# prsinha1/Distributed-Inverse-Problem-Admm

Hardware: AMD Instinct MI355X
Metric: ADMM node-updates/sec (whole node), 512² phantom; rel-Fro vs CPU ref (higher is better)
Workload: dtype f32 samples / f64 state; 1 GPU; C3 (BASELINE.json configs[2] 512^2, 16 graph nodes (ring), 96 angles/node, float32 samples, iso TV, lam=0.02 rho=2, split-Bregman 10x5 CG) on 1 GPU(s), one step = one outer ADMM iteration; image=512, nodes=16, angles_per_node=96, graph=ring, parallelism=graph-node shards x1, batch_streams=1

## Files before the change

### distributed-inverse-problem-admm_amd/csrc/admm_tomo.hip

```cpp
#include <hip/hip_runtime.h>

#include <algorithm>
#include <cmath>
#include <cstdio>
#include <cstdlib>
#include <cstring>
#include <string>
#include <type_traits>
#include <utility>
#include <vector>

#include "../../include/admm_tomo.h"
#include "kernels.hpp"

using namespace admm;

namespace {
thread_local std::string g_err;

int fail(int code, const std::string& msg) {
  g_err = msg;
  return code;
}

// ... 64 lines not shown
  double Kb = 0.0;
  int kbias = 0;
  int wexp = 0;
  FgGroup* groups = nullptr;
  FgRange* rng = nullptr;
  int n_groups = 0;
  static constexpr int kPlans = 6;
  FgGroup* plan_groups[kPlans] = {};
  FgRange* plan_rng[kPlans] = {};
  int plan_n[kPlans] = {}, plan_blocks[kPlans] = {};
  double plan_staged[kPlans] = {};
  std::vector<int4> plan_blk[kPlans];
  std::vector<char> plan_caseA[kPlans];
  bool mirror_half = false;
  Buf fg_order;
  int fg_nblk = 0, fg_order_nch = 0;
  int fg_cpb = 1;
  hipStream_t cap = nullptr;

  bool csr = false;
  long long nnz = 0;
  Buf f_ptr, f_idx, f_val, t_ptr, t_idx, t_val;

  Buf op_img, op_imgT, op_sino, op_fpart;
  Buf op_order[kPlans];
  int op_nblk[kPlans] = {};
  int op_fpart_key = -1;

  bool bound = false;
  admm_batch b{};
  int vb = 1;
  bool mm = false;
  int bk_staging = 0;
  int n_cu = 0;
  admm_ctx* half = nullptr;
  Buf xs, xsT, p, pT, Hp, sino, bI, fpart, r, c, d2, e2;
  Buf dsumS;
  Buf x2, p2;
  Buf pring;
  Buf ats;
  std::vector<hipEvent_t>* tf_ev = nullptr;
  size_t tf_next = 0;
  int tf_kind = 0;
  bool ats_valid = false;
  hipGraph_t g_update_reuse = nullptr;
  hipGraphExec_t x_update_reuse = nullptr;
  Buf partH, partS, partD, partE;
  Buf redH;
  int P_back = 0, P_tile = 0, P_fwd = 0, P_edge = 0;
  hipGraph_t g_update = nullptr, g_cons = nullptr;
  hipGraphExec_t x_update = nullptr, x_cons = nullptr;
};

namespace {

#define RET(expr)                   \
  do {                              \
    int _rc = (expr);               \
    if (_rc != ADMM_OK) return _rc; \
  } while (0)

constexpr int kXcds = 8;

int vb_for(int V, int dtype) {
  const int vb = V >= 5 ? 8 : (V >= 3 ? 4 : (V == 2 ? 2 : 1));
  return dtype == ADMM_DTYPE_F64 ? std::min(vb, 4) : vb;
// ... 260 lines not shown
  }
  dim3 cg((C->mrays + kBlock - 1) / kBlock, nch);
  hipLaunchKernelGGL((k_fwd_combine<T, VB, MODE>), cg, dim3(kBlock), 0, s, (const T*)C->fpart.p, sino, b, part,
                     C->fang, C->g.n_det, C->g.n_angles, V);
  CHECK_LAUNCH();
  return ADMM_OK;
}

template <typename T, int VB, int MODE>
int launch_back(admm_ctx* C, BackArgs<T> a, int V, hipStream_t s) {
  if constexpr (MODE == BACK_H || MODE == BACK_INIT || MODE == BACK_DIAG || MODE == BACK_ATB) {
    if (C->mm) {
      constexpr int VBV = mirror_vb<T, VB>(), MH = VBV / 2;
      const admm_ctx* H = C->half;
      a.ang = H->bang;
      a.angc = H->bangc;
      a.K = H->Kb;
      a.kbias = H->kbias;
      a.wexp = H->wexp;
      a.N = C->g.N;
      a.n_det = C->g.n_det;
      a.n_ang = H->g.n_angles;
      a.V = V;
      const int N = C->g.N, Nh = (N + 1) / 2;
      dim3 grid((N + kBTJ - 1) / kBTJ, (Nh + kBTI - 1) / kBTI, ((V + VB - 1) / VB) * (VB / MH));
      bool done = false;
      if constexpr (back_mirror_dma<T, VBV, MODE>()) {
        if (C->bk_staging == 1) {
          hipLaunchKernelGGL((k_back_mirror_reg<T, VBV, VB, MODE>), grid, dim3(kBkThreads), 0, s, a);
          done = true;
        } else if constexpr (std::is_same<T, float>::value && ADMM_BK_LB2) {
          const bool fills = (long)grid.x * grid.y * grid.z >= 2L * C->n_cu;
          if (grid.z % 2 == 0 && (C->bk_staging == 3 || (C->bk_staging == 0 && fills))) {
            hipLaunchKernelGGL((k_back_mirror_2<T, VBV, VB>), dim3(grid.x, grid.y, grid.z / 2), dim3(kBkThreads), 0,
                               s, a);
            done = true;
          }
        }
      }
      if (!done) hipLaunchKernelGGL((k_back_mirror<T, VBV, VB, MODE>), grid, dim3(kBkThreads), 0, s, a);
      CHECK_LAUNCH();
      return ADMM_OK;
    }
  }
  a.ang = C->bang;
  a.angc = C->bangc;
  a.K = C->Kb;
  a.kbias = C->kbias;
  a.wexp = C->wexp;
  a.N = C->g.N;
  a.n_det = C->g.n_det;
  a.n_ang = C->g.n_angles;
  a.V = V;
  const int N = C->g.N;
  dim3 grid((N + kBTJ - 1) / kBTJ, (N + kBTI - 1) / kBTI, MODE == BACK_WSQ ? 1 : (V + VB - 1) / VB);
  if (C->csr) {
    a.csr_ptr = (const int*)C->t_ptr.p;
    a.csr_idx = (const int*)C->t_idx.p;
    a.csr_val = (const T*)C->t_val.p;
    hipLaunchKernelGGL((k_back<T, VB, MODE, true>), grid, dim3(kBkThreads), 0, s, a);
  } else {
    hipLaunchKernelGGL((k_back<T, VB, MODE>), grid, dim3(kBkThreads), 0, s, a);
  }
  CHECK_LAUNCH();
  return ADMM_OK;
}

int back_partitions(admm_ctx* C) {
// ... 344 lines not shown
}

extern "C" {

int admm_abi_version(void) { return ADMM_ABI_VERSION; }
const char* admm_last_error(void) { return g_err.c_str(); }

int admm_ctx_create(admm_ctx** out, const admm_geom* geom, int dtype, int max_images, int device) {
  if (!out || !geom) return fail(ADMM_E_INVALID, "null argument");
  *out = nullptr;
  const admm_geom g = *geom;
  if (g.N < 2 || g.n_angles < 1 || g.n_det < 1) return fail(ADMM_E_INVALID, "bad geometry sizes");
  if (g.N > 4096) return fail(ADMM_E_INVALID, "N > 4096 is not supported");
  if (dtype != ADMM_DTYPE_F32 && dtype != ADMM_DTYPE_F64) return fail(ADMM_E_INVALID, "bad dtype");
  if (max_images < 1) return fail(ADMM_E_INVALID, "max_images < 1");
  const double h = 2.0 / g.N;
  const double hd = (g.det_max - g.det_min) / g.n_det;
  if (!(hd > 0)) return fail(ADMM_E_INVALID, "det_max <= det_min");
  if (hd < h * (1.0 - 1e-9))
    return fail(ADMM_E_INVALID, "detector spacing finer than the pixel size is not supported "
                                "(det_width_factor must be >= 1 with n_det = N)");
  const size_t npix = (size_t)g.N * g.N, m = (size_t)g.n_angles * g.n_det;
  if ((size_t)max_images * npix * 8 >= (1ull << 31) || (size_t)max_images * m * 8 >= (1ull << 31))
    return fail(ADMM_E_INVALID, "batch too large for 32-bit buffer offsets; split it across contexts");
  DEVICE_SCOPE(device);
  admm_ctx* C = new admm_ctx();
  C->g = g;
  C->dtype = dtype;
  C->device = device;
  {
    const char* st = getenv("ADMM_BK_STAGING");
    const std::string v = st ? st : "";
    C->bk_staging = v == "reg" ? 1 : v == "dma1" ? 2 : v == "dma2" ? 3 : 0;
  }
  HIPCHK(hipDeviceGetAttribute(&C->n_cu, hipDeviceAttributeMultiprocessorCount, device));
  C->max_images = max_images;
  C->npix = (int)npix;
  C->mrays = (int)m;

  std::vector<FwdAngle> fa(g.n_angles);
  std::vector<BackAngle> ba(g.n_angles);
  std::vector<BackAngleC> bc(g.n_angles);
  C->Kb = -g.det_min / hd - 0.5;
  const double c0 = 0.5 * (g.N - 1);
  for (int t = 0; t < g.n_angles; ++t) {
    const double th = g.angle_min + (t + 0.5) * (g.angle_max - g.angle_min) / g.n_angles;
    const double cs = std::cos(th), sn = std::sin(th);
    const bool caseA = std::fabs(cs) >= std::fabs(sn);
    const double al = caseA ? cs : sn, be = caseA ? sn : cs;
    fa[t].A0 = c0 + (g.det_min / h + 0.5 * hd / h + c0 * be) / al;
    fa[t].A1 = (hd / h) / al;
    fa[t].dl = -be / al;
    fa[t].L = h / std::fabs(al);
    fa[t].caseA = caseA ? 1 : 0;
    ba[t].Bi = cs * h / hd;
    ba[t].Bj = sn * h / hd;
    ba[t].B0 = -c0 * (ba[t].Bi + ba[t].Bj) - g.det_min / hd - 0.5;
    ba[t].slope = (hd / h) / std::fabs(al);
    ba[t].L = h / std::fabs(al);
    bc[t].Bi = ba[t].Bi;
    bc[t].Bj = ba[t].Bj;
    const float sLf = (float)(ba[t].slope * ba[t].L);
    bc[t].ws = float2v{-sLf, sLf};
    bc[t].wc = float2v{(float)ba[t].L, (float)(ba[t].L - ba[t].slope * ba[t].L)};
    while (std::ldexp((double)bc[t].wc.x, -C->wexp) > 1.0) ++C->wexp;
    const double kmn = C->Kb - c0 * (std::fabs(ba[t].Bi) + std::fabs(ba[t].Bj));
// ... 406 lines not shown
  RET(ensure(C->dsumS, Vp * npix * ds));
  RET(ensure(C->x2, (size_t)V * npix * 8));
  RET(ensure(C->p2, Vp * npix * ds));
  if (B.cg_iters > 1 && B.cg_iters <= kMaxCgRing)
    RET(ensure(C->pring, (size_t)(B.cg_iters - 1) * Vp * npix * ds));
  if (B.flags & ADMM_BATCH_KEEP_X) RET(ensure(C->ats, Vp * npix * ds));
  C->ats_valid = false;
  RET(ensure(C->sino, Vp * m * ds));
  RET(ensure(C->bI, Vp * m * ds));
  RET(ensure(C->r, V * npix * 8));
  RET(ensure(C->c, V * npix * 8));
  RET(ensure(C->d2, 2 * V * npix * 8));
  RET(ensure(C->e2, 2 * V * npix * 8));
  C->P_back = back_partitions(C);
  const int N = C->g.N;
  C->P_tile = ((N + kTile - 1) / kTile) * ((N + kTile - 1) / kTile);
  if ((size_t)Vp * npix * ds >= (1ull << 31) || (size_t)Vp * m * ds >= (1ull << 31))
    return fail(ADMM_E_INVALID, "batch too large for 32-bit buffer offsets");
  C->P_fwd = C->mm ? (int)((C->half->mrays + kBlock - 1) / kBlock)
           : (C->n_groups > 0 || C->csr) ? (int)((m + kBlock - 1) / kBlock)
                                         : ((C->g.n_det + kFwdRays - 1) / kFwdRays) * C->g.n_angles;
  C->P_edge = B.z ? (int)((npix + kBlock * 4 - 1) / (kBlock * 4)) : (int)((npix + kConsPix - 1) / kConsPix);
  RET(ensure(C->partH, (size_t)5 * V * C->P_back * 8));
  RET(ensure(C->partS, (size_t)V * C->P_fwd * 8));
  RET(ensure(C->partD, (size_t)5 * V * C->P_back * 8));
  RET(ensure(C->partE, (size_t)3 * std::max(1, B.n_edges) * C->P_edge * 8));
  RET(ensure(C->redH, (size_t)5 * V * 8 * std::max(1, std::min(B.cg_iters, kMaxCgRing))));
  C->bound = true;
  RET(with_vb(C->vb, [&](auto vbc) {
    constexpr int VB = decltype(vbc)::value;
    const int nch = (V + VB - 1) / VB;
    if (C->dtype == ADMM_DTYPE_F32)
      hipLaunchKernelGGL((k_pack_d<float, VB>), dim3((unsigned)((npix + 255) / 256), nch), dim3(256), 0, C->cap,
                         B.dsum, (float*)C->dsumS.p, (int)npix, V);
    else
      hipLaunchKernelGGL((k_pack_d<double, VB>), dim3((unsigned)((npix + 255) / 256), nch), dim3(256), 0, C->cap,
                         B.dsum, (double*)C->dsumS.p, (int)npix, V);
    CHECK_LAUNCH();
    return ADMM_OK;
  }));
  HIPCHK(hipStreamSynchronize(C->cap));
  auto fu = [&](hipStream_t s) {
    return C->dtype == ADMM_DTYPE_F32 ? enqueue_update_any<float>(C, s) : enqueue_update_any<double>(C, s);
  };
  RET(capture(C, fu, &C->g_update, &C->x_update));
  if (B.flags & ADMM_BATCH_KEEP_X) {
    auto fr = [&](hipStream_t s) {
      return C->dtype == ADMM_DTYPE_F32 ? enqueue_update_any<float>(C, s, true)
                                        : enqueue_update_any<double>(C, s, true);
    };
    RET(capture(C, fr, &C->g_update_reuse, &C->x_update_reuse));
  }
  if (B.n_edges > 0) {
    auto fc = [&](hipStream_t s) { return enqueue_consensus(C, s); };
    RET(capture(C, fc, &C->g_cons, &C->x_cons));
  }
  HIPCHK(hipDeviceSynchronize());
  return ADMM_OK;
}

extern "C++" {
template <typename T>
int batch_atb(admm_ctx* C, double* atb_out, hipStream_t s) {
  const int V = C->b.V;
  return with_vb(C->vb, [&](auto vbc) {
    constexpr int VB = decltype(vbc)::value;
    const int nch = (V + VB - 1) / VB;
    hipLaunchKernelGGL((k_pack<T, VB>), dim3((C->mrays + 255) / 256, nch), dim3(256), 0, s, (const T*)C->b.b,
                       (T*)C->bI.p, C->mrays, V);
    CHECK_LAUNCH();
// ... 172 lines not shown
```

### distributed-inverse-problem-admm_amd/csrc/kernels.hpp

```cpp
#pragma once
#include <hip/hip_runtime.h>
#include <stdint.h>

#include <type_traits>

namespace admm {

constexpr int kBlock = 256;
constexpr int kTile = 32;
constexpr int kFwdRays = 64;
constexpr int kFwdSegs = 8;
constexpr int kFwdBlock = kFwdRays * kFwdSegs;

struct FwdAngle {
  double A0, A1, dl;
  double L;
  int caseA;
  int pad;
};
struct BackAngle {
  double B0, Bi, Bj;
  double slope, L;
};

// ... 1064 lines not shown
  const double c = x[i * N + j];
  gx = (i < N - 1) ? x[(i + 1) * N + j] - c : 0.0;
  gy = (j < N - 1) ? x[i * N + j + 1] - c : 0.0;
}

__device__ __forceinline__ void tv_sub(double gx, double gy, int kind, double& px, double& py) {
  if (kind == 0) {
    const double m = sqrt(gx * gx + gy * gy);
    if (m > 1e-12) {
      px = gx / m;
      py = gy / m;
    } else {
      px = 0.0;
      py = 0.0;
    }
  } else {
    px = fabs(gx) > 1e-12 ? copysign(1.0, gx) : 0.0;
    py = fabs(gy) > 1e-12 ? copysign(1.0, gy) : 0.0;
  }
}

__device__ __forceinline__ double kt_w_at(const double* __restrict__ d, const double* __restrict__ e, int N,
                                          int i, int j) {
  const int n = N * N;
  double s = 0.0;
  const int o = i * N + j;
  if (i >= 1) s += d[o - N] - e[o - N];
  if (i <= N - 2) s -= d[o] - e[o];
  if (j >= 1) s += d[n + o - 1] - e[n + o - 1];
  if (j <= N - 2) s -= d[n + o] - e[n + o];
  return s;
}

template <typename T, int VB, int MODE, int NQ, int VS = VB, bool ACC = false>
__device__ __forceinline__ void back_epilogue(const BackArgs<T>& A, int i, int j, int chunk, int v0, int nv,
                                              const T (&acc)[VB], double (&pq)[VB][NQ], int lo = 0) {
  const int N = A.N;
  const int npix = N * N;
  const int pix = i * N + j;
  const size_t sbase = (size_t)chunk * npix * VS + lo;
  if constexpr (MODE == BACK_PLAIN) {
    gstore<T, VB>(A.out_t + sbase + (size_t)pix * VS, acc);
  } else if constexpr (MODE == BACK_ATB) {
#pragma unroll
    for (int u = 0; u < VB; ++u)
      if (u < nv) A.out_d[(size_t)(v0 + u) * npix + pix] = (double)acc[u];
  } else if constexpr (MODE == BACK_WSQ) {
    A.out_d[pix] = fmax((double)acc[0], 1e-12);
  } else if constexpr (MODE == BACK_H && std::is_same<T, float>::value) {
    using F2 = float2v;
    constexpr int NP = VB / 2;
    const T* pv = A.pin + sbase;
    T pc[VB], pn[VB], dv[VB], outv[VB];
    F2 kt2[NP > 0 ? NP : 1], pc2[NP > 0 ? NP : 1];
    float kt1 = 0.0f;
    gload<T, VB>(pv + (size_t)pix * VS, pc);
#pragma unroll
    for (int h = 0; h < NP; ++h) {
      pc2[h] = F2{pc[2 * h], pc[2 * h + 1]};
      kt2[h] = F2{0.0f, 0.0f};
    }
    auto nb = [&](size_t o, bool sub_pc_first) {
      gload<T, VB>(pv + o * VS, pn);
#pragma unroll
      for (int h = 0; h < NP; ++h) {
        const F2 q = F2{pn[2 * h], pn[2 * h + 1]};
        kt2[h] = sub_pc_first ? kt2[h] + (pc2[h] - q) : kt2[h] - (q - pc2[h]);
      }
      if constexpr (VB % 2) kt1 = sub_pc_first ? kt1 + (pc[VB - 1] - pn[VB - 1]) : kt1 - (pn[VB - 1] - pc[VB - 1]);
    };
    if (i >= 1) nb((size_t)(pix - N), true);
    if (i <= N - 2) nb((size_t)(pix + N), false);
    if (j >= 1) nb((size_t)(pix - 1), true);
    if (j <= N - 2) nb((size_t)(pix + 1), false);
    gload<T, VB>(A.dsum_s + sbase + (size_t)pix * VS, dv);
    const float rf = (float)A.rho, mf = (float)A.mu;
    const F2 rho2 = F2{rf, rf}, mu2 = F2{mf, mf};
#pragma unroll
    for (int h = 0; h < NP; ++h) {
      const F2 d2 = F2{dv[2 * h], dv[2 * h + 1]} * rho2;
      F2 hv = __builtin_elementwise_fma(d2, pc2[h], F2{acc[2 * h], acc[2 * h + 1]});
      hv = __builtin_elementwise_fma(mu2, kt2[h], hv);
      outv[2 * h] = hv.x;
      outv[2 * h + 1] = hv.y;
    }
    if constexpr (VB % 2) outv[VB - 1] = fmaf(mf, kt1, fmaf(dv[VB - 1] * rf, pc[VB - 1], acc[VB - 1]));
#pragma unroll
    for (int u = 0; u < VB; ++u) {
      if (u >= nv) outv[u] = T(0);
      if (u < nv) {
        const double hd = (double)outv[u], pcd = (double)pc[u];
        const double rv = A.r[(size_t)(v0 + u) * npix + pix];
        pq[u][0] = fma(pcd, hd, ACC ? pq[u][0] : 0.0);
        pq[u][1] = fma(rv, hd, ACC ? pq[u][1] : 0.0);
        pq[u][2] = fma(hd, hd, ACC ? pq[u][2] : 0.0);
        pq[u][3] = fma(rv, rv, ACC ? pq[u][3] : 0.0);
        pq[u][4] = fma(rv, pcd, ACC ? pq[u][4] : 0.0);
      }
    }
    gstore<T, VB>(A.out_t + sbase + (size_t)pix * VS, outv);
  } else if constexpr (MODE == BACK_H || MODE == BACK_INIT) {
    const T* pv = A.pin + sbase;
    T pc[VB], pn[VB];
    double ktk[VB];
    gload<T, VB>(pv + (size_t)pix * VS, pc);
    if (i >= 1) {
      gload<T, VB>(pv + (size_t)(pix - N) * VS, pn);
#pragma unroll
      for (int u = 0; u < VB; ++u) ktk[u] = (double)pc[u] - (double)pn[u];
    } else {
#pragma unroll
      for (int u = 0; u < VB; ++u) ktk[u] = 0.0;
    }
    if (i <= N - 2) {
      gload<T, VB>(pv + (size_t)(pix + N) * VS, pn);
#pragma unroll
      for (int u = 0; u < VB; ++u) ktk[u] -= (double)pn[u] - (double)pc[u];
    }
    if (j >= 1) {
      gload<T, VB>(pv + (size_t)(pix - 1) * VS, pn);
#pragma unroll
      for (int u = 0; u < VB; ++u) ktk[u] += (double)pc[u] - (double)pn[u];
    }
    if (j <= N - 2) {
      gload<T, VB>(pv + (size_t)(pix + 1) * VS, pn);
#pragma unroll
      for (int u = 0; u < VB; ++u) ktk[u] -= (double)pn[u] - (double)pc[u];
    }
    T outv[VB], dv[VB];
    if constexpr (MODE == BACK_H) gload<T, VB>(A.dsum_s + sbase + (size_t)pix * VS, dv);
#pragma unroll
    for (int u = 0; u < VB; ++u) {
      outv[u] = T(0);
      if (u < nv) {
        const size_t vo = (size_t)(v0 + u) * npix;
        const double pcd = (double)pc[u];
        const double dd = (MODE == BACK_H) ? (double)dv[u] : A.dsum[vo + pix];
        const double h = (double)acc[u] + A.rho * dd * pcd + A.mu * ktk[u];
        if constexpr (MODE == BACK_H) {
          const T hp = (T)h;
          outv[u] = hp;
          const double hd = (double)hp;
          const double rv = A.r[vo + pix];
          if constexpr (ACC) {
            pq[u][0] += pcd * hd;
            pq[u][1] += rv * hd;
            pq[u][2] += hd * hd;
            pq[u][3] += rv * rv;
            pq[u][4] += rv * pcd;
          } else {
            pq[u][0] = pcd * hd;
            pq[u][1] = rv * hd;
            pq[u][2] = hd * hd;
            pq[u][3] = rv * rv;
            pq[u][4] = rv * pcd;
          }
        } else {
          const double* dv = A.dvar + 2 * vo;
          const double* ev = A.evar + 2 * vo;
          const double rr = A.atb[vo + pix] + A.rho * A.cvec[vo + pix] + A.mu * kt_w_at(dv, ev, N, i, j) - h;
          A.out_d[vo + pix] = rr;
          outv[u] = (T)rr;
        }
      }
    }
    gstore<T, VB>(A.out_t + sbase + (size_t)pix * VS, outv);
  }
}

#ifndef ADMM_BK_TI
#define ADMM_BK_TI 32
// ... 347 lines not shown
  for (int u = 0; u < VB; ++u)
#pragma unroll
    for (int q = 0; q < NQ; ++q) pq[u][q] = 0.0;
  if constexpr (MODE == BACK_DIAG) {
    __shared__ double diag_s[kDiagScratch];
    diag_epilogue_tile<T, VB>(A, diag_s, ib, jb, i, j, inb, chunk, v0, nv, acc, pq);
  } else if (inb) {
    back_epilogue<T, VB, MODE, NQ>(A, i, j, chunk, v0, nv, acc, pq);
  }

  if constexpr (MODE == BACK_H || MODE == BACK_DIAG) {
    constexpr int NT = VB * NQ, NS = RsShape<NT>::NS;
    __shared__ double lds[kBkWaves * NS];
    __shared__ double tot[NS];
    double flat[NT];
#pragma unroll
    for (int u = 0; u < VB; ++u)
#pragma unroll
      for (int q = 0; q < NQ; ++q) flat[u * NQ + q] = pq[u][q];
    block_reduce_flat<NT, kBkWaves>(flat, lds, tot);
    const int t = threadIdx.x;
    if (t < VB * NQ && t / NQ < nv) {
      const int P = gridDim.x * gridDim.y;
      const int b = blockIdx.y * gridDim.x + blockIdx.x;
      A.part[((size_t)v0 * NQ + t) * P + b] = tot[t];
    }
  }
}

template <typename T, int VB, int MODE>
constexpr bool back_mirror_dma() {
  return ADMM_BK_DMA && MODE == BACK_H && Planes<T, VB>::NPL == 2 && sizeof(Pack<T, Planes<T, VB>::PV>) == 16;
}
template <typename T, int VB, int VBR, int MODE, bool DMAQ>
__device__ __forceinline__ void back_mirror_body(const BackArgs<T>& A) {
  static_assert(MODE == BACK_H || MODE == BACK_INIT || MODE == BACK_DIAG || MODE == BACK_ATB, "batch modes");
  constexpr int MH = VB / 2, MS = VBR / MH;
  static_assert(VB % 2 == 0 && VBR % MH == 0, "mirror: VB = 2 x (a divisor of VBR)");
  constexpr int NQ = (MODE == BACK_H || MODE == BACK_DIAG) ? 5 : 1;
  constexpr int NPL = Planes<T, VB>::NPL, PV = Planes<T, VB>::PV;
  constexpr int PB = (int)sizeof(Pack<T, PV>);
  const int N = A.N, n_det = A.n_det, n_ang = A.n_ang;
  const int Nh = (N + 1) / 2;
  const size_t m_full = (size_t)2 * n_ang * n_det;
  const int jb = blockIdx.x * kBTJ, ib = blockIdx.y * kBTI;
  const int lane = threadIdx.x & 63, wv = threadIdx.x >> 6;
  const int j = jb + 16 * (wv % kBkPatchJ) + (lane & 15);
  const int i = ib + 4 * (wv / kBkPatchJ) + (lane >> 4);
  const int i2 = N - 1 - i;
  const bool inb = (i < Nh) && (j < N);
  const bool inb2 = inb && (i2 != i);
  const int chunk = blockIdx.z, rc = chunk / MS, mq = chunk % MS;
  const int v0 = rc * VBR + mq * MH;
  const int nv = min(MH, A.V - v0);
  const double c0 = 0.5 * (N - 1);
  const double xi = (double)min(i, Nh - 1) - c0, yj = (double)min(j, N - 1) - c0;
  const int jhi = min(jb + kBTJ - 1, N - 1), ihi = min(ib + kBTI - 1, Nh - 1);
  const int kbias = A.kbias;
  const double Kc = A.K + (double)kbias;
  const double Kcb = Kc + kKfBias;
  constexpr bool FB = std::is_same<T, float>::value;
  constexpr int ANGC_ = ((NPL > 2) ? kBAngC / 2 : kBAngC) / 2;
  constexpr int ANGC_DIAG = (98304 / (2 * NPL * kBWin * PB)) & ~3;
  constexpr int ANGC = (MODE == BACK_DIAG && ANGC_ > ANGC_DIAG) ? ANGC_DIAG : ANGC_;
  static_assert(ANGC % 4 == 0 && ANGC >= 4, "angle chunks are read as int4 groups");
  constexpr bool DMA = DMAQ && back_mirror_dma<T, VB, MODE>();
  constexpr int NWB = DMA ? 4 : 2, NKS = DMA ? 3 : 2;
  constexpr int BUFB = 2 * NPL * ANGC * kBWin * PB;
  __shared__ Pack<T, PV> win[NWB][NPL][ANGC][kBWin];
  __shared__ int4 kmin_s[NKS][2][ANGC / 4 + 1];
  __shared__ int kst_s[DMA ? 3 : 1][2][DMA ? ANGC + 1 : 1];
  T acc1[VB], acc2[VB];
#pragma unroll
  for (int u = 0; u < VB; ++u) acc1[u] = acc2[u] = T(0);
  const T* sino_c = A.sino + (size_t)rc * m_full * VBR + mq * MH;
  int t0c = 0;

  auto kmin_load = [&](int t0) {
    const BackAngleC& g = A.angc[min(t0 + ((int)threadIdx.x % ANGC), n_ang - 1)];
    return make_double2(g.Bi, g.Bj);
  };
  auto kmin_store = [&](int buf, double2 bij, int bo = 0) {
    const int w = (int)threadIdx.x / ANGC;
    const double xa = (double)ib - c0, xb = (double)ihi - c0;
    const double x0 = w ? -xb : xa, x1 = w ? -xa : xb;
    auto kf = [&](double xx, int jj) { return fma(xx, bij.x, fma((double)jj - c0, bij.y, Kc)); };
    const double kmn = fmin(fmin(kf(x0, jb), kf(x0, jhi)), fmin(kf(x1, jb), kf(x1, jhi)));
    const int a = (int)threadIdx.x % ANGC;
    const int k0w = (int)floor(kmn) - 1;
    int koff = (a * kBWin - k0w) * PB;
    if constexpr (FB) koff = (int)((unsigned)koff - kKfHi * (unsigned)PB);
    if constexpr (DMA) {
      koff = (int)((unsigned)koff + (unsigned)bo);
      kst_s[buf][min(w, 1)][w < 2 ? a : ANGC] = k0w - kbias;
    }
    reinterpret_cast<int*>(kmin_s[buf][min(w, 1)])[w < 2 ? a : ANGC] = koff;
  };
  auto kmin_chunk = [&](int t0, int buf) { kmin_store(buf, kmin_load(t0)); };
  auto kmin_chunk_b = [&](int t0, int buf, int bo) { kmin_store(buf, kmin_load(t0), bo); };
  constexpr int NE = 2 * ANGC * kBWin * NPL;
  constexpr int SPER = (NE + kBkThreads - 1) / kBkThreads;
// ... 178 lines not shown
      chunk_taps(t0, nt, kb);
      if (t0 + ANGC < n_ang) {
        __syncthreads();
        wcommit(t0 + ANGC);
        kmin_store(kb, rec2);
        __syncthreads();
      }
    }
  }
  if constexpr (std::is_same<T, float>::value) {
    if (A.wexp != 0) {
#pragma unroll
      for (int u = 0; u < VB; ++u) {
        acc1[u] = ldexpf(acc1[u], A.wexp);
        acc2[u] = ldexpf(acc2[u], A.wexp);
      }
    }
  }
  T r1[MH], r2[MH];
#pragma unroll
  for (int h = 0; h < MH; ++h) {
    r1[h] = acc1[h] + acc2[MH + h];
    r2[h] = acc2[h] + acc1[MH + h];
  }
  double pq[MH][NQ];
#pragma unroll
  for (int u = 0; u < MH; ++u)
#pragma unroll
    for (int q = 0; q < NQ; ++q) pq[u][q] = 0.0;
  if constexpr (MODE == BACK_DIAG) {
    __shared__ double diag_s[kDiagScratch];
    diag_epilogue_tile<T, MH, VBR>(A, diag_s, ib, jb, i, j, inb, rc, v0, nv, r1, pq, mq * MH);
    diag_epilogue_tile<T, MH, VBR>(A, diag_s, N - ib - kBTI, jb, i2, j, inb2, rc, v0, nv, r2, pq, mq * MH);
  } else {
    if (inb) back_epilogue<T, MH, MODE, NQ, VBR>(A, i, j, rc, v0, nv, r1, pq, mq * MH);
    if (inb2) back_epilogue<T, MH, MODE, NQ, VBR, true>(A, i2, j, rc, v0, nv, r2, pq, mq * MH);
  }
  if constexpr (MODE == BACK_H || MODE == BACK_DIAG) {
    constexpr int NT = MH * NQ, NS = RsShape<NT>::NS;
    __shared__ double lds[kBkWaves * NS];
    __shared__ double tot[NS];
    double flat[NT];
#pragma unroll
    for (int u = 0; u < MH; ++u)
#pragma unroll
      for (int q = 0; q < NQ; ++q) flat[u * NQ + q] = pq[u][q];
    block_reduce_flat<NT, kBkWaves>(flat, lds, tot);
    const int t = threadIdx.x;
    if (t < MH * NQ && t / NQ < nv) {
      const int P = gridDim.x * gridDim.y;
      const int b = blockIdx.y * gridDim.x + blockIdx.x;
      A.part[((size_t)v0 * NQ + t) * P + b] = tot[t];
    }
  }
}

template <typename T, int VB, int VBR, int MODE>
__global__ __launch_bounds__(kBkThreads) void k_back_mirror(BackArgs<T> A) {
  back_mirror_body<T, VB, VBR, MODE, true>(A);
}
template <typename T, int VB, int VBR, int MODE>
__global__ __launch_bounds__(kBkThreads) void k_back_mirror_reg(BackArgs<T> A) {
  back_mirror_body<T, VB, VBR, MODE, false>(A);
}

template <typename T, int VB, int VBR>
__global__ __launch_bounds__(kBkThreads) void k_back_mirror_2(BackArgs<T> A) {
  constexpr int MODE = BACK_H, NQ = 5, LB = 2;
  constexpr int MH = VB / 2, MS = VBR / MH;
  static_assert(VB % 2 == 0 && VBR % MH == 0, "mirror: VB = 2 x (a divisor of VBR)");
  constexpr int NPL = Planes<T, VB>::NPL, PV = Planes<T, VB>::PV;
  constexpr int PB = (int)sizeof(Pack<T, PV>);
  static_assert(std::is_same<T, float>::value && NPL == 2 && PB == 16, "float32 16-byte window packs");
  const int N = A.N, n_det = A.n_det, n_ang = A.n_ang;
  const int Nh = (N + 1) / 2;
  const size_t m_full = (size_t)2 * n_ang * n_det;
  const int jb = blockIdx.x * kBTJ, ib = blockIdx.y * kBTI;
  const int lane = threadIdx.x & 63, wv = threadIdx.x >> 6;
  const int j = jb + 16 * (wv % kBkPatchJ) + (lane & 15);
  const int i = ib + 4 * (wv / kBkPatchJ) + (lane >> 4);
  const int i2 = N - 1 - i;
  const bool inb = (i < Nh) && (j < N);
  const bool inb2 = inb && (i2 != i);
  const double c0 = 0.5 * (N - 1);
  const double xi = (double)min(i, Nh - 1) - c0, yj = (double)min(j, N - 1) - c0;
  const int jhi = min(jb + kBTJ - 1, N - 1), ihi = min(ib + kBTI - 1, Nh - 1);
  const int kbias = A.kbias;
  const double Kc = A.K + (double)kbias;
  const double Kcb = Kc + kKfBias;
  constexpr int ANGC = kBAngC / 4;
  static_assert(ANGC % 4 == 0 && ANGC >= 4, "angle chunks are read as int4 groups");
  constexpr int WINB = 2 * NPL * ANGC * kBWin * PB;
  constexpr int BUFB = LB * WINB;
  __shared__ Pack<T, PV> win[2 * LB * 2][NPL][ANGC][kBWin];
  __shared__ int4 kmin_s[3][2][ANGC / 4 + 1];
  __shared__ int kst_s[3][2][ANGC + 1];
  T acc1[LB][VB], acc2[LB][VB];
#pragma unroll
  for (int l = 0; l < LB; ++l)
#pragma unroll
    for (int u = 0; u < VB; ++u) acc1[l][u] = acc2[l][u] = T(0);

  auto kmin_load = [&](int t0) {
    const BackAngleC& g = A.angc[min(t0 + ((int)threadIdx.x % ANGC), n_ang - 1)];
    return make_double2(g.Bi, g.Bj);
  };
  auto kmin_store = [&](int ks, double2 bij, int bo) {
    const int w = (int)threadIdx.x / ANGC;
    const double xa = (double)ib - c0, xb = (double)ihi - c0;
    const double x0 = w ? -xb : xa, x1 = w ? -xa : xb;
    auto kf = [&](double xx, int jj) { return fma(xx, bij.x, fma((double)jj - c0, bij.y, Kc)); };
    const double kmn = fmin(fmin(kf(x0, jb), kf(x0, jhi)), fmin(kf(x1, jb), kf(x1, jhi)));
    const int a = (int)threadIdx.x % ANGC;
    const int k0w = (int)floor(kmn) - 1;
    const int koff = (int)((unsigned)((a * kBWin - k0w) * PB) - kKfHi * (unsigned)PB + (unsigned)bo);
    kst_s[ks][min(w, 1)][w < 2 ? a : ANGC] = k0w - kbias;
    reinterpret_cast<int*>(kmin_s[ks][min(w, 1)])[w < 2 ? a : ANGC] = koff;
  };
  constexpr int NE = LB * 2 * ANGC * kBWin * NPL;
  constexpr int NI = NE / (64 * kBkWaves);
  static_assert(NE % (64 * kBkWaves) == 0 && (ANGC * kBWin) % 64 == 0, "whole pieces, one (lane block, window, plane) each");
  const int wvu = __builtin_amdgcn_readfirstlane(wv);
  auto dma = [&](int t0, int ks, int bo) {
    const int nt = min(ANGC, n_ang - t0);
#pragma unroll
    for (int e = 0; e < NI; ++e) {
// ... 64 lines not shown
#pragma unroll
      for (int u = 0; u < 4; ++u) g[u] = rec(gq + u);
      const int4 k1 = kmin_s[ks][0][tt >> 2], k2 = kmin_s[ks][1][tt >> 2];
      tap2(g[0], k1.x, k2.x);
      tap2(g[1], k1.y, k2.y);
      tap2(g[2], k1.z, k2.z);
      tap2(g[3], k1.w, k2.w);
    }
    for (; tt < nt; ++tt)
      tap2(rec(gq + (tt & 3)), reinterpret_cast<const int*>(kmin_s[ks][0])[tt],
           reinterpret_cast<const int*>(kmin_s[ks][1])[tt]);
  };
  kmin_store(0, kmin_load(0), 0);
  if (ANGC < n_ang) kmin_store(1, kmin_load(ANGC), BUFB);
  __syncthreads();
  dma(0, 0, 0);
  __syncthreads();
  for (int t0 = 0, ci = 0, ks = 0; t0 < n_ang; t0 += ANGC, ++ci, ks = ks == 2 ? 0 : ks + 1) {
    const int nt = min(ANGC, n_ang - t0);
    const double2 rec2 = kmin_load(min(t0 + 2 * ANGC, n_ang - 1));
    const int ks1 = ks == 2 ? 0 : ks + 1, ks2 = ks1 == 2 ? 0 : ks1 + 1;
    if (t0 + ANGC < n_ang) dma(t0 + ANGC, ks1, (ci & 1) ? 0 : BUFB);
    chunk_taps(t0, nt, ks);
    if (t0 + ANGC < n_ang) {
      if (t0 + 2 * ANGC < n_ang) kmin_store(ks2, rec2, (ci & 1) ? BUFB : 0);
      __syncthreads();
    }
  }
  constexpr int NT = MH * NQ, NS = RsShape<NT>::NS;
  __shared__ double lds[kBkWaves * NS];
  __shared__ double tot[NS];
  const int P = gridDim.x * gridDim.y;
  const int b = blockIdx.y * gridDim.x + blockIdx.x;
#pragma unroll
  for (int l = 0; l < LB; ++l) {
    if (A.wexp != 0) {
#pragma unroll
      for (int u = 0; u < VB; ++u) {
        acc1[l][u] = ldexpf(acc1[l][u], A.wexp);
        acc2[l][u] = ldexpf(acc2[l][u], A.wexp);
      }
    }
    T r1[MH], r2[MH];
#pragma unroll
    for (int h = 0; h < MH; ++h) {
      r1[h] = acc1[l][h] + acc2[l][MH + h];
      r2[h] = acc2[l][h] + acc1[l][MH + h];
    }
    double pq[MH][NQ];
#pragma unroll
    for (int u = 0; u < MH; ++u)
#pragma unroll
      for (int q = 0; q < NQ; ++q) pq[u][q] = 0.0;
    const int z = (int)blockIdx.z * LB + l, rc = z / MS, mq = z % MS;
    const int v0 = rc * VBR + mq * MH, nv = min(MH, A.V - v0);
    if (inb) back_epilogue<T, MH, MODE, NQ, VBR>(A, i, j, rc, v0, nv, r1, pq, mq * MH);
    if (inb2) back_epilogue<T, MH, MODE, NQ, VBR, true>(A, i2, j, rc, v0, nv, r2, pq, mq * MH);
    double flat[NT];
#pragma unroll
    for (int u = 0; u < MH; ++u)
#pragma unroll
      for (int q = 0; q < NQ; ++q) flat[u * NQ + q] = pq[u][q];
    block_reduce_flat<NT, kBkWaves>(flat, lds, tot);
    const int t = threadIdx.x;
    if (t < NT && t / NQ < nv) A.part[((size_t)v0 * NQ + t) * P + b] = tot[t];
  }
}

template <int VB>
struct EwMap {
  static constexpr int TI = kTile / VB;
  static constexpr int RPI = 8 / VB;
  int u, jj, isub;
  __device__ EwMap() : u(threadIdx.x % VB), jj((threadIdx.x / VB) % kTile), isub(threadIdx.x / (kTile * VB)) {}
};

template <typename T, int VB>
struct TileT {
  T t[EwMap<VB>::TI][kTile + 1][VB];
};

template <typename T, int VB>
__device__ __forceinline__ void tile_store_T(TileT<T, VB>& tl, T* __restrict__ outT, int N, int i0, int j0) {
  constexpr int TI = EwMap<VB>::TI;
  __syncthreads();
  const int u = threadIdx.x % VB, r = (threadIdx.x / VB) % TI, c0 = threadIdx.x / (VB * TI);
  for (int c = c0; c < kTile; c += kBlock / (VB * TI)) {
    const int jj = j0 + c, ii = i0 + r;
    if (jj < N && ii < N) outT[((size_t)jj * N + ii) * VB + u] = tl.t[r][c][u];
  }
}

template <typename T, int VB>
__global__ __launch_bounds__(kBlock) void k_start_reuse(
    const T* __restrict__ ats, const double* __restrict__ x, EdgeIn E, const double* __restrict__ q,
    const int* __restrict__ inc_off, const int* __restrict__ inc_edge, const int* __restrict__ inc_qslot,
    const int* __restrict__ inc_sign, const double* __restrict__ atb, double* __restrict__ cvec,
    const double* __restrict__ dsum, const double* __restrict__ dvar, const double* __restrict__ evar,
    double* __restrict__ r, T* __restrict__ p, T* __restrict__ pT, double rho, double mu, int N, int V) {
  constexpr int ROWS = kBlock / kTile;
  __shared__ T tl[ROWS][kTile + 1][VB];
  const int chunk = blockIdx.z, v0 = chunk * VB, nv = min(VB, V - v0);
  const int npix = N * N;
  const size_t sbase = (size_t)chunk * npix * VB;
  const int jj = threadIdx.x % kTile, ii = threadIdx.x / kTile;
  const int i0 = blockIdx.y * ROWS, j0 = blockIdx.x * kTile;
  const int i = i0 + ii, j = j0 + jj;
  if (i < N && j < N) {
    const int pix = i * N + j;
    T av[VB], outv[VB];
    gload<T, VB>(ats + sbase + (size_t)pix * VB, av);
#pragma unroll
    for (int u = 0; u < VB; ++u) {
      outv[u] = T(0);
      if (u < nv) {
        const int v = v0 + u;
        const size_t vo = (size_t)v * npix;
        const double* xv = x + vo;
        double cc = 0.0;
        for (int qq = inc_off[v]; qq < inc_off[v + 1]; ++qq) {
          const double vij = edge_v(E, inc_edge[qq], inc_sign[qq], npix, pix);
          cc += q[(size_t)inc_qslot[qq] * npix + pix] * vij;
        }
        cvec[vo + pix] = cc;
        const double pcd = (double)(T)xv[pix];
        double ktk = 0.0;
        if (i >= 1) ktk += pcd - (double)(T)xv[pix - N];
        if (i <= N - 2) ktk -= (double)(T)xv[pix + N] - pcd;
        if (j >= 1) ktk += pcd - (double)(T)xv[pix - 1];
        if (j <= N - 2) ktk -= (double)(T)xv[pix + 1] - pcd;
        const double ab = atb[vo + pix];
        const double h = ((double)av[u] + ab) + rho * dsum[vo + pix] * pcd + mu * ktk;
        const double rr = ab + rho * cc + mu * kt_w_at(dvar + 2 * vo, evar + 2 * vo, N, i, j) - h;
        r[vo + pix] = rr;
        outv[u] = (T)rr;
      }
      tl[ii][jj][u] = outv[u];
    }
    gstore<T, VB>(p + sbase + (size_t)pix * VB, outv);
  }
  __syncthreads();
  const int u = threadIdx.x % VB, rr_ = (threadIdx.x / VB) % ROWS, c0 = threadIdx.x / (VB * ROWS);
  for (int c = c0; c < kTile; c += kBlock / (VB * ROWS)) {
    const int jc = j0 + c, ic = i0 + rr_;
    if (jc < N && ic < N) pT[sbase + ((size_t)jc * N + ic) * VB + u] = tl[rr_][c][u];
  }
}

template <typename T, int VB>
__global__ __launch_bounds__(kBlock) void k_gather(const double* __restrict__ x, EdgeIn E,
                                                   const double* __restrict__ q,
                                                   const int* __restrict__ inc_off, const int* __restrict__ inc_edge,
                                                   const int* __restrict__ inc_qslot,
                                                   const int* __restrict__ inc_sign, double* __restrict__ c,
                                                   T* __restrict__ xs, T* __restrict__ xsT, int N, int V) {
  __shared__ TileT<T, VB> tl;
  const EwMap<VB> mp;
  const int chunk = blockIdx.z, v = chunk * VB + mp.u;
  const bool live = v < V;
  const int npix = N * N;
  const size_t sbase = (size_t)chunk * npix * VB;
  const int i0 = blockIdx.y * EwMap<VB>::TI, j0 = blockIdx.x * kTile;
  const int e0 = live ? inc_off[v] : 0, e1 = live ? inc_off[v + 1] : 0;
// ... 316 lines not shown
    T sv = T(0);
    if (live) {
      double gx, gy, ux, uy, ndx, ndy, e0, e1;
      if constexpr (UIN) {
        const double u0 = din[2 * vo + o], u1 = din[2 * vo + npix + o];
        double d0, d1;
        shrink2(u0, u1, tau, kind, d0, d1);
        e0 = u0 - d0;
        e1 = u1 - d1;
      } else {
        e0 = ev[o];
        e1 = ev[npix + o];
      }
      gradx(mp.u, xv, i, j, gx, gy);
      ux = gx + e0;
      uy = gy + e1;
      shrink2(ux, uy, tau, kind, ndx, ndy);
      const double nex = ux - ndx, ney = uy - ndy;
      dout[2 * vo + o] = ndx;
      dout[2 * vo + npix + o] = ndy;
      eout[2 * vo + o] = nex;
      eout[2 * vo + npix + o] = ney;
      const double xn = xat(mp.u, xv, i, j);
      if constexpr (FUSE) xout[vo + o] = xn;
      sv = (T)xn;
    }
    p[sbase + (size_t)o * VB + mp.u] = sv;
    tl.t[rw][mp.jj][mp.u] = sv;
  }
  tv_tile_store_T<T, VB>(tl, pT + sbase, N, i0, j0);
}

template <typename T, int VB>
__global__ void k_pack_d(const double* __restrict__ in, T* __restrict__ out, int L, int V) {
  const int q = blockIdx.x * blockDim.x + threadIdx.x;
  const int chunk = blockIdx.y, v0 = chunk * VB;
  if (q >= L) return;
  T s[VB];
#pragma unroll
  for (int u = 0; u < VB; ++u) s[u] = (v0 + u < V) ? (T)in[(size_t)(v0 + u) * L + q] : T(0);
  gstore<T, VB>(out + ((size_t)chunk * L + q) * VB, s);
}

template <typename T, int VB>
__global__ void k_pack(const T* __restrict__ in, T* __restrict__ out, int L, int V) {
  const int q = blockIdx.x * blockDim.x + threadIdx.x;
  const int chunk = blockIdx.y, v0 = chunk * VB;
  if (q >= L) return;
  T s[VB];
#pragma unroll
  for (int u = 0; u < VB; ++u) s[u] = (v0 + u < V) ? in[(size_t)(v0 + u) * L + q] : T(0);
  gstore<T, VB>(out + ((size_t)chunk * L + q) * VB, s);
}

template <typename T, int VB>
__global__ void k_unpack(const T* __restrict__ in, T* __restrict__ out, int L, int V) {
  const int q = blockIdx.x * blockDim.x + threadIdx.x;
  const int chunk = blockIdx.y, v0 = chunk * VB;
  if (q >= L) return;
  T s[VB];
  gload<T, VB>(in + ((size_t)chunk * L + q) * VB, s);
#pragma unroll
  for (int u = 0; u < VB; ++u)
    if (v0 + u < V) out[(size_t)(v0 + u) * L + q] = s[u];
}

template <bool WEIGHTED>
__global__ __launch_bounds__(kBlock) void k_consensus(const double* __restrict__ xext, double* __restrict__ y,
                                                      double* __restrict__ yb, double* __restrict__ z,
                                                      const double* __restrict__ w,
                                                      const int* __restrict__ ea, const int* __restrict__ eb,
                                                      double* __restrict__ part, int npix, int e0 = 0) {
  __shared__ double lds[12];
// ... 177 lines not shown
```

Before: 2237 node-updates/s.

## Stage backprojection epilogue p-tiles and start-reuse x halos in LDS; prescale dsum by rho

```diff
diff --git a/distributed-inverse-problem-admm_amd/csrc/admm_tomo.hip b/distributed-inverse-problem-admm_amd/csrc/admm_tomo.hip
--- a/distributed-inverse-problem-admm_amd/csrc/admm_tomo.hip
+++ b/distributed-inverse-problem-admm_amd/csrc/admm_tomo.hip
@@ -120,6 +120,7 @@
   int vb = 1;
   bool mm = false;
   int bk_staging = 0;
+  bool bk_epi_lds = true;
   int n_cu = 0;
   admm_ctx* half = nullptr;
   Buf xs, xsT, p, pT, Hp, sino, bI, fpart, r, c, d2, e2;
@@ -446,8 +447,18 @@
         } else if constexpr (std::is_same<T, float>::value && ADMM_BK_LB2) {
           const bool fills = (long)grid.x * grid.y * grid.z >= 2L * C->n_cu;
           if (grid.z % 2 == 0 && (C->bk_staging == 3 || (C->bk_staging == 0 && fills))) {
-            hipLaunchKernelGGL((k_back_mirror_2<T, VBV, VB>), dim3(grid.x, grid.y, grid.z / 2), dim3(kBkThreads), 0,
-                               s, a);
+            if (C->bk_epi_lds)
+              hipLaunchKernelGGL((k_back_mirror_2<T, VBV, VB>), dim3(grid.x, grid.y, grid.z / 2),
+                                 dim3(kBkThreads), 0, s, a);
+            else
+              hipLaunchKernelGGL((k_back_mirror_2_gepi<T, VBV, VB>), dim3(grid.x, grid.y, grid.z / 2),
+                                 dim3(kBkThreads), 0, s, a);
+            done = true;
+          }
+        }
+        if constexpr (std::is_same<T, float>::value) {
+          if (!done && !C->bk_epi_lds) {
+            hipLaunchKernelGGL((k_back_mirror_gepi<T, VBV, VB, MODE>), grid, dim3(kBkThreads), 0, s, a);
             done = true;
           }
         }
@@ -858,6 +869,8 @@
     const char* st = getenv("ADMM_BK_STAGING");
     const std::string v = st ? st : "";
     C->bk_staging = v == "reg" ? 1 : v == "dma1" ? 2 : v == "dma2" ? 3 : 0;
+    const char* ep = getenv("ADMM_BK_EPI");
+    C->bk_epi_lds = !(ep && std::string(ep) == "global");
   }
   HIPCHK(hipDeviceGetAttribute(&C->n_cu, hipDeviceAttributeMultiprocessorCount, device));
   C->max_images = max_images;
@@ -1330,10 +1343,10 @@
     const int nch = (V + VB - 1) / VB;
     if (C->dtype == ADMM_DTYPE_F32)
       hipLaunchKernelGGL((k_pack_d<float, VB>), dim3((unsigned)((npix + 255) / 256), nch), dim3(256), 0, C->cap,
-                         B.dsum, (float*)C->dsumS.p, (int)npix, V);
+                         B.dsum, (float*)C->dsumS.p, (int)npix, V, B.rho);
     else
       hipLaunchKernelGGL((k_pack_d<double, VB>), dim3((unsigned)((npix + 255) / 256), nch), dim3(256), 0, C->cap,
-                         B.dsum, (double*)C->dsumS.p, (int)npix, V);
+                         B.dsum, (double*)C->dsumS.p, (int)npix, V, B.rho);
     CHECK_LAUNCH();
     return ADMM_OK;
   }));
diff --git a/distributed-inverse-problem-admm_amd/csrc/kernels.hpp b/distributed-inverse-problem-admm_amd/csrc/kernels.hpp
--- a/distributed-inverse-problem-admm_amd/csrc/kernels.hpp
+++ b/distributed-inverse-problem-admm_amd/csrc/kernels.hpp
@@ -1120,9 +1120,24 @@
   return s;
 }
 
-template <typename T, int VB, int MODE, int NQ, int VS = VB, bool ACC = false>
+struct PGlobal {};
+template <typename T, int VB, int PITCH>
+struct PTile {
+  static_assert(sizeof(Pack<T, VB>) == 16, "one 16-byte slot per pixel");
+  const __attribute__((address_space(3))) char* base;
+  int i0, j0;
+  __device__ __forceinline__ void load(int i, int j, T (&o)[VB]) const {
+    typedef unsigned int u32x4 __attribute__((ext_vector_type(4)));
+    const u32x4 k =
+        *reinterpret_cast<const __attribute__((address_space(3))) u32x4*>(base + ((i - i0) * PITCH + (j - j0)) * 16);
+    __builtin_memcpy(o, &k, 16);
+  }
+};
+
+template <typename T, int VB, int MODE, int NQ, int VS = VB, bool ACC = false, class PSrc = PGlobal>
 __device__ __forceinline__ void back_epilogue(const BackArgs<T>& A, int i, int j, int chunk, int v0, int nv,
-                                              const T (&acc)[VB], double (&pq)[VB][NQ], int lo = 0) {
+                                              const T (&acc)[VB], double (&pq)[VB][NQ], int lo = 0,
+                                              PSrc psrc = PSrc{}) {
   const int N = A.N;
   const int npix = N * N;
   const int pix = i * N + j;
@@ -1142,14 +1157,20 @@
     T pc[VB], pn[VB], dv[VB], outv[VB];
     F2 kt2[NP > 0 ? NP : 1], pc2[NP > 0 ? NP : 1];
     float kt1 = 0.0f;
-    gload<T, VB>(pv + (size_t)pix * VS, pc);
+    auto ldp = [&](int ii, int jj, T(&o)[VB]) {
+      if constexpr (std::is_same<PSrc, PGlobal>::value)
+        gload<T, VB>(pv + (size_t)(ii * N + jj) * VS, o);
+      else
+        psrc.load(ii, jj, o);
+    };
+    ldp(i, j, pc);
 #pragma unroll
     for (int h = 0; h < NP; ++h) {
       pc2[h] = F2{pc[2 * h], pc[2 * h + 1]};
       kt2[h] = F2{0.0f, 0.0f};
     }
-    auto nb = [&](size_t o, bool sub_pc_first) {
-      gload<T, VB>(pv + o * VS, pn);
+    auto nb = [&](int ii, int jj, bool sub_pc_first) {
+      ldp(ii, jj, pn);
 #pragma unroll
       for (int h = 0; h < NP; ++h) {
         const F2 q = F2{pn[2 * h], pn[2 * h + 1]};
@@ -1157,22 +1178,22 @@
       }
       if constexpr (VB % 2) kt1 = sub_pc_first ? kt1 + (pc[VB - 1] - pn[VB - 1]) : kt1 - (pn[VB - 1] - pc[VB - 1]);
     };
-    if (i >= 1) nb((size_t)(pix - N), true);
-    if (i <= N - 2) nb((size_t)(pix + N), false);
-    if (j >= 1) nb((size_t)(pix - 1), true);
-    if (j <= N - 2) nb((size_t)(pix + 1), false);
+    if (i >= 1) nb(i - 1, j, true);
+    if (i <= N - 2) nb(i + 1, j, false);
+    if (j >= 1) nb(i, j - 1, true);
+    if (j <= N - 2) nb(i, j + 1, false);
     gload<T, VB>(A.dsum_s + sbase + (size_t)pix * VS, dv);
-    const float rf = (float)A.rho, mf = (float)A.mu;
-    const F2 rho2 = F2{rf, rf}, mu2 = F2{mf, mf};
+    const float mf = (float)A.mu;
+    const F2 mu2 = F2{mf, mf};
 #pragma unroll
     for (int h = 0; h < NP; ++h) {
-      const F2 d2 = F2{dv[2 * h], dv[2 * h + 1]} * rho2;
+      const F2 d2 = F2{dv[2 * h], dv[2 * h + 1]};
       F2 hv = __builtin_elementwise_fma(d2, pc2[h], F2{acc[2 * h], acc[2 * h + 1]});
       hv = __builtin_elementwise_fma(mu2, kt2[h], hv);
       outv[2 * h] = hv.x;
       outv[2 * h + 1] = hv.y;
     }
-    if constexpr (VB % 2) outv[VB - 1] = fmaf(mf, kt1, fmaf(dv[VB - 1] * rf, pc[VB - 1], acc[VB - 1]));
+    if constexpr (VB % 2) outv[VB - 1] = fmaf(mf, kt1, fmaf(dv[VB - 1], pc[VB - 1], acc[VB - 1]));
 #pragma unroll
     for (int u = 0; u < VB; ++u) {
       if (u >= nv) outv[u] = T(0);
@@ -1223,8 +1244,8 @@
       if (u < nv) {
         const size_t vo = (size_t)(v0 + u) * npix;
         const double pcd = (double)pc[u];
-        const double dd = (MODE == BACK_H) ? (double)dv[u] : A.dsum[vo + pix];
-        const double h = (double)acc[u] + A.rho * dd * pcd + A.mu * ktk[u];
+        const double rd = (MODE == BACK_H) ? (double)dv[u] : A.rho * A.dsum[vo + pix];
+        const double h = (double)acc[u] + rd * pcd + A.mu * ktk[u];
         if constexpr (MODE == BACK_H) {
           const T hp = (T)h;
           outv[u] = hp;
@@ -1638,7 +1659,39 @@
 constexpr bool back_mirror_dma() {
   return ADMM_BK_DMA && MODE == BACK_H && Planes<T, VB>::NPL == 2 && sizeof(Pack<T, Planes<T, VB>::PV>) == 16;
 }
-template <typename T, int VB, int VBR, int MODE, bool DMAQ>
+constexpr int kPtR = kBTI + 2, kPtC = kBTJ + 2, kPtSlots = kPtR * kPtC;
+using lds_char = __attribute__((address_space(3))) char;
+template <int LB>
+constexpr int ptile_bytes() {
+  return ((2 * LB * kPtSlots + 63) / 64) * 64 * 16;
+}
+template <typename T, int VBR, int MH, int LB>
+__device__ __forceinline__ void ptile_stage(const BackArgs<T>& A, lds_char* lds, int ib, int jb, int z0) {
+  static_assert(MH * sizeof(T) == 16, "one 16-byte slot per pixel and lane block");
+  constexpr int MS = VBR / MH, NSLOT = 2 * LB * kPtSlots, NPC = (NSLOT + 63) / 64;
+  const int N = A.N, npix = N * N;
+  const int lane = threadIdx.x & 63;
+  const int wvu = __builtin_amdgcn_readfirstlane((int)threadIdx.x >> 6);
+  const uint64_t b = (uint64_t)(uintptr_t)A.pin;
+  const uint32_t lo = __builtin_amdgcn_readfirstlane((uint32_t)b);
+  const uint32_t hi = __builtin_amdgcn_readfirstlane((uint32_t)(b >> 32));
+  const __amdgpu_buffer_rsrc_t rs =
+      make_rsrc((const void*)(uintptr_t)(((uint64_t)hi << 32) | lo),
+                (uint32_t)((size_t)((A.V + VBR - 1) / VBR) * npix * VBR * sizeof(T)));
+  for (int pc = wvu; pc < NPC; pc += kBkWaves) {
+    const int q = pc * 64 + lane;
+    const int t = q / kPtSlots, s = q - t * kPtSlots, rr = s / kPtC, cc = s - rr * kPtC;
+    const int z = z0 + (t >> 1);
+    const int row = ((t & 1) ? N - 1 - ib - kBTI : ib - 1) + rr, col = jb - 1 + cc;
+    const bool in = q < NSLOT && row >= 0 && row < N && col >= 0 && col < N;
+    const unsigned voff =
+        in ? (unsigned)(((z / MS) * npix + row * N + col) * VBR + (z % MS) * MH) * (unsigned)sizeof(T) : 0xFFFFFFFFu;
+    __builtin_amdgcn_raw_ptr_buffer_load_lds(rs, (__attribute__((address_space(3))) void*)(lds + pc * (64 * 16)), 16,
+                                             voff, 0, 0, 0);
+  }
+}
+
+template <typename T, int VB, int VBR, int MODE, bool DMAQ, bool EPIQ = true>
 __device__ __forceinline__ void back_mirror_body(const BackArgs<T>& A) {
   static_assert(MODE == BACK_H || MODE == BACK_INIT || MODE == BACK_DIAG || MODE == BACK_ATB, "batch modes");
   constexpr int MH = VB / 2, MS = VBR / MH;
@@ -1673,6 +1726,8 @@
   constexpr bool DMA = DMAQ && back_mirror_dma<T, VB, MODE>();
   constexpr int NWB = DMA ? 4 : 2, NKS = DMA ? 3 : 2;
   constexpr int BUFB = 2 * NPL * ANGC * kBWin * PB;
+  constexpr bool EPI = EPIQ && DMA && std::is_same<T, float>::value && MH * sizeof(T) == 16;
+  static_assert(!EPI || ptile_bytes<1>() <= 2 * BUFB, "the p tiles fit in the window array");
   __shared__ Pack<T, PV> win[NWB][NPL][ANGC][kBWin];
   __shared__ int4 kmin_s[NKS][2][ANGC / 4 + 1];
   __shared__ int kst_s[DMA ? 3 : 1][2][DMA ? ANGC + 1 : 1];
@@ -1917,6 +1972,17 @@
     __shared__ double diag_s[kDiagScratch];
     diag_epilogue_tile<T, MH, VBR>(A, diag_s, ib, jb, i, j, inb, rc, v0, nv, r1, pq, mq * MH);
     diag_epilogue_tile<T, MH, VBR>(A, diag_s, N - ib - kBTI, jb, i2, j, inb2, rc, v0, nv, r2, pq, mq * MH);
+  } else if constexpr (EPI) {
+    lds_char* const tb = (lds_char*)&win[0][0][0][0];
+    __syncthreads();
+    ptile_stage<T, VBR, MH, 1>(A, tb, ib, jb, chunk);
+    asm volatile("s_waitcnt vmcnt(0)" ::: "memory");
+    __syncthreads();
+    using PT = PTile<T, MH, kPtC>;
+    if (inb) back_epilogue<T, MH, MODE, NQ, VBR, false, PT>(A, i, j, rc, v0, nv, r1, pq, mq * MH, PT{tb, ib - 1, jb - 1});
+    if (inb2)
+      back_epilogue<T, MH, MODE, NQ, VBR, true, PT>(A, i2, j, rc, v0, nv, r2, pq, mq * MH,
+                                                    PT{tb + kPtSlots * 16, N - 1 - ib - kBTI, jb - 1});
   } else {
     if (inb) back_epilogue<T, MH, MODE, NQ, VBR>(A, i, j, rc, v0, nv, r1, pq, mq * MH);
     if (inb2) back_epilogue<T, MH, MODE, NQ, VBR, true>(A, i2, j, rc, v0, nv, r2, pq, mq * MH);
@@ -1948,9 +2014,13 @@
 __global__ __launch_bounds__(kBkThreads) void k_back_mirror_reg(BackArgs<T> A) {
   back_mirror_body<T, VB, VBR, MODE, false>(A);
 }
-
-template <typename T, int VB, int VBR>
-__global__ __launch_bounds__(kBkThreads) void k_back_mirror_2(BackArgs<T> A) {
+template <typename T, int VB, int VBR, int MODE>
+__global__ __launch_bounds__(kBkThreads) void k_back_mirror_gepi(BackArgs<T> A) {
+  back_mirror_body<T, VB, VBR, MODE, true, false>(A);
+}
+
+template <typename T, int VB, int VBR, bool EPI>
+__device__ __forceinline__ void back_mirror_2_body(const BackArgs<T>& A) {
   constexpr int MODE = BACK_H, NQ = 5, LB = 2;
   constexpr int MH = VB / 2, MS = VBR / MH;
   static_assert(VB % 2 == 0 && VBR % MH == 0, "mirror: VB = 2 x (a divisor of VBR)");
@@ -1977,6 +2047,7 @@
   static_assert(ANGC % 4 == 0 && ANGC >= 4, "angle chunks are read as int4 groups");
   constexpr int WINB = 2 * NPL * ANGC * kBWin * PB;
   constexpr int BUFB = LB * WINB;
+  static_assert(!EPI || (MH * sizeof(T) == 16 && ptile_bytes<LB>() <= 2 * BUFB), "the p tiles fit in the window array");
   __shared__ Pack<T, PV> win[2 * LB * 2][NPL][ANGC][kBWin];
   __shared__ int4 kmin_s[3][2][ANGC / 4 + 1];
   __shared__ int kst_s[3][2][ANGC + 1];
@@ -2107,6 +2178,13 @@
   __shared__ double tot[NS];
   const int P = gridDim.x * gridDim.y;
   const int b = blockIdx.y * gridDim.x + blockIdx.x;
+  lds_char* const tb = (lds_char*)&win[0][0][0][0];
+  if constexpr (EPI) {
+    __syncthreads();
+    ptile_stage<T, VBR, MH, LB>(A, tb, ib, jb, (int)blockIdx.z * LB);
+    asm volatile("s_waitcnt vmcnt(0)" ::: "memory");
+    __syncthreads();
+  }
 #pragma unroll
   for (int l = 0; l < LB; ++l) {
     if (A.wexp != 0) {
@@ -2129,8 +2207,18 @@
       for (int q = 0; q < NQ; ++q) pq[u][q] = 0.0;
     const int z = (int)blockIdx.z * LB + l, rc = z / MS, mq = z % MS;
     const int v0 = rc * VBR + mq * MH, nv = min(MH, A.V - v0);
-    if (inb) back_epilogue<T, MH, MODE, NQ, VBR>(A, i, j, rc, v0, nv, r1, pq, mq * MH);
-    if (inb2) back_epilogue<T, MH, MODE, NQ, VBR, true>(A, i2, j, rc, v0, nv, r2, pq, mq * MH);
+    if constexpr (EPI) {
+      using PT = PTile<T, MH, kPtC>;
+      if (inb)
+        back_epilogue<T, MH, MODE, NQ, VBR, false, PT>(A, i, j, rc, v0, nv, r1, pq, mq * MH,
+                                                       PT{tb + (2 * l) * kPtSlots * 16, ib - 1, jb - 1});
+      if (inb2)
+        back_epilogue<T, MH, MODE, NQ, VBR, true, PT>(A, i2, j, rc, v0, nv, r2, pq, mq * MH,
+                                                      PT{tb + (2 * l + 1) * kPtSlots * 16, N - 1 - ib - kBTI, jb - 1});
+    } else {
+      if (inb) back_epilogue<T, MH, MODE, NQ, VBR>(A, i, j, rc, v0, nv, r1, pq, mq * MH);
+      if (inb2) back_epilogue<T, MH, MODE, NQ, VBR, true>(A, i2, j, rc, v0, nv, r2, pq, mq * MH);
+    }
     double flat[NT];
 #pragma unroll
     for (int u = 0; u < MH; ++u)
@@ -2140,6 +2228,14 @@
     const int t = threadIdx.x;
     if (t < NT && t / NQ < nv) A.part[((size_t)v0 * NQ + t) * P + b] = tot[t];
   }
+}
+template <typename T, int VB, int VBR>
+__global__ __launch_bounds__(kBkThreads) void k_back_mirror_2(BackArgs<T> A) {
+  back_mirror_2_body<T, VB, VBR, true>(A);
+}
+template <typename T, int VB, int VBR>
+__global__ __launch_bounds__(kBkThreads) void k_back_mirror_2_gepi(BackArgs<T> A) {
+  back_mirror_2_body<T, VB, VBR, false>(A);
 }
 
 template <int VB>
@@ -2166,6 +2262,9 @@
   }
 }
 
+#ifndef ADMM_SR_LDS
+#define ADMM_SR_LDS 1
+#endif
 template <typename T, int VB>
 __global__ __launch_bounds__(kBlock) void k_start_reuse(
     const T* __restrict__ ats, const double* __restrict__ x, EdgeIn E, const double* __restrict__ q,
@@ -2181,6 +2280,35 @@
   const int jj = threadIdx.x % kTile, ii = threadIdx.x / kTile;
   const int i0 = blockIdx.y * ROWS, j0 = blockIdx.x * kTile;
   const int i = i0 + ii, j = j0 + jj;
+#if ADMM_SR_LDS
+  __shared__ T xt[VB][ROWS + 2][kTile + 2];
+  {
+    constexpr int NIN = (ROWS + 2) * kTile, NEL = (ROWS + 2) * (kTile + 2);
+    constexpr int PER = (NEL + kBlock - 1) / kBlock;
+    double xl[VB][PER];
+#pragma unroll
+    for (int u = 0; u < VB; ++u)
+#pragma unroll
+      for (int e = 0; e < PER; ++e) {
+        const int q = (int)threadIdx.x + e * kBlock;
+        const int rr = q < NIN ? q / kTile : (q - NIN) >> 1;
+        const int cc = q < NIN ? 1 + q % kTile : ((q - NIN) & 1) * (kTile + 1);
+        const int row = i0 - 1 + rr, col = j0 - 1 + cc;
+        const bool in = q < NEL && u < nv && row >= 0 && row < N && col >= 0 && col < N;
+        xl[u][e] = in ? x[(size_t)(v0 + u) * npix + row * N + col] : 0.0;
+      }
+#pragma unroll
+    for (int u = 0; u < VB; ++u)
+#pragma unroll
+      for (int e = 0; e < PER; ++e) {
+        const int q = (int)threadIdx.x + e * kBlock;
+        const int rr = q < NIN ? q / kTile : (q - NIN) >> 1;
+        const int cc = q < NIN ? 1 + q % kTile : ((q - NIN) & 1) * (kTile + 1);
+        if (q < NEL) xt[u][rr][cc] = (T)xl[u][e];
+      }
+    __syncthreads();
+  }
+#endif
   if (i < N && j < N) {
     const int pix = i * N + j;
     T av[VB], outv[VB];
@@ -2191,19 +2319,28 @@
       if (u < nv) {
         const int v = v0 + u;
         const size_t vo = (size_t)v * npix;
-        const double* xv = x + vo;
         double cc = 0.0;
         for (int qq = inc_off[v]; qq < inc_off[v + 1]; ++qq) {
           const double vij = edge_v(E, inc_edge[qq], inc_sign[qq], npix, pix);
           cc += q[(size_t)inc_qslot[qq] * npix + pix] * vij;
         }
         cvec[vo + pix] = cc;
+#if ADMM_SR_LDS
+        const double pcd = (double)xt[u][ii + 1][jj + 1];
+        double ktk = 0.0;
+        if (i >= 1) ktk += pcd - (double)xt[u][ii][jj + 1];
+        if (i <= N - 2) ktk -= (double)xt[u][ii + 2][jj + 1] - pcd;
+        if (j >= 1) ktk += pcd - (double)xt[u][ii + 1][jj];
+        if (j <= N - 2) ktk -= (double)xt[u][ii + 1][jj + 2] - pcd;
+#else
+        const double* xv = x + vo;
         const double pcd = (double)(T)xv[pix];
         double ktk = 0.0;
         if (i >= 1) ktk += pcd - (double)(T)xv[pix - N];
         if (i <= N - 2) ktk -= (double)(T)xv[pix + N] - pcd;
         if (j >= 1) ktk += pcd - (double)(T)xv[pix - 1];
         if (j <= N - 2) ktk -= (double)(T)xv[pix + 1] - pcd;
+#endif
         const double ab = atb[vo + pix];
         const double h = ((double)av[u] + ab) + rho * dsum[vo + pix] * pcd + mu * ktk;
         const double rr = ab + rho * cc + mu * kt_w_at(dvar + 2 * vo, evar + 2 * vo, N, i, j) - h;
@@ -2586,13 +2723,14 @@
 }
 
 template <typename T, int VB>
-__global__ void k_pack_d(const double* __restrict__ in, T* __restrict__ out, int L, int V) {
+__global__ void k_pack_d(const double* __restrict__ in, T* __restrict__ out, int L, int V, double scale) {
   const int q = blockIdx.x * blockDim.x + threadIdx.x;
   const int chunk = blockIdx.y, v0 = chunk * VB;
   if (q >= L) return;
+  const T sc = (T)scale;
   T s[VB];
 #pragma unroll
-  for (int u = 0; u < VB; ++u) s[u] = (v0 + u < V) ? (T)in[(size_t)(v0 + u) * L + q] : T(0);
+  for (int u = 0; u < VB; ++u) s[u] = (v0 + u < V) ? (T)in[(size_t)(v0 + u) * L + q] * sc : T(0);
   gstore<T, VB>(out + ((size_t)chunk * L + q) * VB, s);
 }
 
```

After: 2262 node-updates/s, median of 6. +1.1%, better.
